# ZhongchuanSun/scikit-recommender

Measured on AMD Instinct MI355X. Metric: train interactions/sec + eval users/sec (HR@10/NDCG@10) at 1/2/4/8 MI355X, higher is better.
Workload: dtype f32; 1 GPU; BASELINE configs[1]: BPRMF d=64, synthetic 1000000-user/100000-item/50000000-interaction (MovieLens-shaped), exact-stream sampler + fused BPR step + dense Adam; eval = fused MFMA top-10; users=1000000, items=100000, train_interactions=48383462, batch_per_gpu=1024, global_batch=1024

## Files before the change

scikit-recommender_amd/csrc/bpr_fused.hip:

```cpp
#include "adam_math.h"

#include <cstdlib>

using namespace skr;

namespace {

constexpr int BPR_WAVES = 4;

constexpr int FUSED_SLOT_BITS = 20;
constexpr int FUSED_PRE = 7;

struct FusedRow {
    float p, m, v, g;
};

__device__ __forceinline__ void fused_advance(FusedRow& r, int prev1, int s_from, int s_to, const AdamBlockArgs& a, int ck) {
    if (prev1 > 0)
        adam_grad_run(r.p, r.g, r.m, r.v, a, prev1 - 1, s_to, ck);
    else
        adam_zero_run(r.p, r.m, r.v, a, s_from, s_to, ck);
}

struct FusedWork {
    float *wp, *wm, *wv, *g;
    int64_t cap;
};

__global__ __launch_bounds__(BPR_WAVES * 64) void bpr_fused_step_kernel(
    const float* __restrict__ P, const float* __restrict__ M, const float* __restrict__ V, int64_t n_par, FusedWork w,
    const int32_t* __restrict__ u_ids, const int32_t* __restrict__ i_ids, const int32_t* __restrict__ j_ids,
    const int32_t* __restrict__ meta, int n, int64_t ublk0, int64_t iblk0, int64_t bblk0, int s_now, AdamBlockArgs a,
    float reg, float* __restrict__ loss, int loss_slots, int dbg, const float* __restrict__ pre) {
    __shared__ float s_loss[BPR_WAVES], s_l2[BPR_WAVES];
    if (!(dbg & 16)) __builtin_amdgcn_s_setprio(3);
    const int lane = threadIdx.x & 63, wv = threadIdx.x >> 6;
    const AdamChainArgs ca = adam_chain_args(a);
    float acc_loss = 0.0f, acc_l2 = 0.0f;
    for (int b = blockIdx.x * BPR_WAVES + wv; b < n; b += gridDim.x * BPR_WAVES) {
        const int64_t u = u_ids[b], i = i_ids[b], j = j_ids[b];
        int32_t mt[5];
        int64_t blk[5] = {ublk0 + u, iblk0 + i, iblk0 + j, bblk0 + (i >> 6), bblk0 + (j >> 6)};
#pragma unroll
        for (int r = 0; r < 5; ++r) mt[r] = __builtin_amdgcn_readfirstlane(meta[static_cast<int64_t>(r) * n + b]);
        FusedRow row[5];
        int from[5];
#pragma unroll
        for (int r = 0; r < 5; ++r) {
            const int64_t slot = mt[r] & ((1 << FUSED_SLOT_BITS) - 1);
            int n0 = (mt[r] >> FUSED_SLOT_BITS) & 7;
            row[r] = FusedRow{1.0f, 0.0f, 0.0f, 0.0f};
            from[r] = (mt[r] >> 24) & 0x7f;
            if (n0 == FUSED_PRE) {
                const int64_t e = slot * 64 + lane;
                row[r].p = pre[e];
                row[r].m = pre[w.cap * 64 + e];
                row[r].v = pre[2 * w.cap * 64 + e];
                from[r] = s_now;
                mt[r] &= ~(7 << FUSED_SLOT_BITS);
                n0 = 0;
            } else if (((mt[r] >> 24) & 0x7f) == 0) {
                const int64_t e = blk[r] * 64 + lane;
                if (e < n_par) {
                    row[r].p = P[e];
                    row[r].m = M[e];
                    row[r].v = V[e];
                }
            } else {
                const int64_t e = ((n0 & 1) * w.cap + slot) * 64 + lane;
                row[r].p = w.wp[e];
                row[r].m = w.wm[e];
                row[r].v = w.wv[e];
                row[r].g = w.g[(((n0 + 2) % 3) * w.cap + slot) * 64 + lane];
            }
        }
        if (!(dbg & 1)) {
#pragma unroll
            for (int r = 0; r < 5; ++r) {
                const int prev1 = (mt[r] >> 24) & 0x7f;
                const AdamRowState o = chain_advance(row[r].p, row[r].g, row[r].m, row[r].v, prev1, from[r], s_now,
                                                     r < 3 ? FC_STEP_ROW : FC_STEP_BIAS, ca);
                row[r].p = o.p, row[r].m = o.m, row[r].v = o.v;
            }
        }
        if (!(dbg & 4)) {
#pragma unroll
            for (int r = 0; r < 5; ++r) {
                if ((mt[r] >> 23) & 1) {
                    const int64_t slot = mt[r] & ((1 << FUSED_SLOT_BITS) - 1);
                    const int n0 = (mt[r] >> FUSED_SLOT_BITS) & 7;
                    const int64_t e = (((n0 + 1) & 1) * w.cap + slot) * 64 + lane;
                    w.wp[e] = row[r].p;
                    w.wm[e] = row[r].m;
                    w.wv[e] = row[r].v;
                    w.g[(((n0 + 1) % 3) * w.cap + slot) * 64 + lane] = 0.0f;
                }
            }
        }
        const float pu = row[0].p, qi = row[1].p, qj = row[2].p;
        const float bi = __shfl(row[3].p, static_cast<int>(i & 63)), bj = __shfl(row[4].p, static_cast<int>(j & 63));
        const float xi = skr::wave_sum(pu * qi) + bi, xj = skr::wave_sum(pu * qj) + bj;
        const float x = xi - xj;
        const float z = expf(-fabsf(x));
        const float l = -(fminf(0.0f, x) - log1pf(z));
        const float sig_neg = (x >= 0.0f) ? z / (1.0f + z) : 1.0f / (1.0f + z);
        const float c = -sig_neg;
        float sq = skr::wave_sum(pu * pu + qi * qi + qj * qj);
        float* gcur[5];
#pragma unroll
        for (int r = 0; r < 5; ++r) {
            const int64_t slot = mt[r] & ((1 << FUSED_SLOT_BITS) - 1);
            const int n0 = (mt[r] >> FUSED_SLOT_BITS) & 7;
            gcur[r] = w.g + ((n0 % 3) * w.cap + slot) * 64;
        }
        if (!(dbg & 2)) {
            const float gu = c * (qi - qj) + reg * pu, gi = c * pu + reg * qi, gj = -c * pu + reg * qj;
            if (mt[0] < 0) gcur[0][lane] = gu; else atomicAdd(&gcur[0][lane], gu);
            if (mt[1] < 0) gcur[1][lane] = gi; else atomicAdd(&gcur[1][lane], gi);
            if (mt[2] < 0) gcur[2][lane] = gj; else atomicAdd(&gcur[2][lane], gj);
        }
        sq += bi * bi + bj * bj;
        if (lane == 0 && !(dbg & 2)) {
            atomicAdd(&gcur[3][i & 63], c + reg * bi);
            atomicAdd(&gcur[4][j & 63], -c + reg * bj);
        }
        acc_loss += l;
        acc_l2 += 0.5f * sq;
    }
    if (lane == 0) {
        s_loss[wv] = acc_loss;
        s_l2[wv] = acc_l2;
    }
    __syncthreads();
    if (threadIdx.x == 0 && !(dbg & 8)) {
        float x = 0.0f, y = 0.0f;
        for (int q = 0; q < BPR_WAVES; ++q) {
            x += s_loss[q];
            y += s_l2[q];
        }
        const int sl = 2 * (static_cast<int>(blockIdx.x) % loss_slots);
        atomicAdd(&loss[sl], x);
        atomicAdd(&loss[sl + 1], y);
    }
}

__global__ __launch_bounds__(256) void bpr_fused_pre_kernel(const float* __restrict__ P, const float* __restrict__ M,
                                                            const float* __restrict__ V, int64_t n_par, float* __restrict__ pre,
                                                            int64_t cap, const int32_t* __restrict__ slot_blk,
                                                            const int32_t* __restrict__ slot_fin, const int32_t* __restrict__ n_slots,
                                                            AdamBlockArgs a, const int32_t* __restrict__ tag_prev,
                                                            int32_t tag_prev_value) {
    const int lane = threadIdx.x & 63;
    const int64_t slot = blockIdx.x * 4 + (threadIdx.x >> 6);
    if (slot >= *n_slots) return;
    const int64_t blk = slot_blk[slot];
    const int first = (slot_fin[slot] >> 16) & 0xff;
    if (first == 0 || tag_prev[blk] == tag_prev_value) return;
    const int64_t e = blk * 64 + lane;
    FusedRow r{1.0f, 0.0f, 0.0f, 0.0f};
    if (e < n_par) { r.p = P[e]; r.m = M[e]; r.v = V[e]; }
    fused_advance(r, 0, 0, first, a, FC_PRE);
    const int64_t o = slot * 64 + lane;
    pre[o] = r.p;
    pre[cap * 64 + o] = r.m;
    pre[2 * cap * 64 + o] = r.v;
}

__global__ __launch_bounds__(256) void bpr_fused_end_kernel(float* __restrict__ P, float* __restrict__ M, float* __restrict__ V,
                                                            int64_t n_par, FusedWork w, const int32_t* __restrict__ slot_blk,
                                                            const int32_t* __restrict__ slot_fin,
                                                            const int32_t* __restrict__ n_slots, AdamBlockArgs a,
                                                            const int32_t* __restrict__ tag_next, int32_t tag_next_value, int which) {
    const int lane = threadIdx.x & 63;
    const int64_t slot0 = 2 * (static_cast<int64_t>(blockIdx.x) * 4 + __builtin_amdgcn_readfirstlane(threadIdx.x >> 6));
    const int64_t n = *n_slots;
    if (slot0 >= n) return;
    FusedRow r[2];
    int64_t e[2];
    int last[2];
    bool live[2];
#pragma unroll
    for (int h = 0; h < 2; ++h) {
        const int64_t slot = slot0 + h;
        live[h] = slot < n;
        e[h] = 0, last[h] = 0;
        r[h] = FusedRow{1.0f, 0.0f, 0.0f, 0.0f};
        if (!live[h]) continue;
        const int64_t blk = slot_blk[slot];
        if (which != 0 && ((tag_next[blk] == tag_next_value) != (which == 1))) {
            live[h] = false;
            continue;
        }
        const int fin = slot_fin[slot], nn = fin & 7;
        last[h] = (fin >> 8) & 0xff;
        e[h] = blk * 64 + lane;
        if (e[h] < n_par) {
            const int64_t o = ((nn & 1) * w.cap + slot) * 64 + lane;
            r[h].p = w.wp[o];
            r[h].m = w.wm[o];
            r[h].v = w.wv[o];
            r[h].g = w.g[(((nn + 2) % 3) * w.cap + slot) * 64 + lane];
        }
    }
    if (live[0] && live[1]) {
        bool ord[2];
#pragma unroll
        for (int h = 0; h < 2; ++h) {
            adam_moments(r[h].g, r[h].m, r[h].v, a);
            ord[h] = __builtin_amdgcn_ballot_w64(!lane_ordinary(r[h].m, r[h].v, a)) == 0;
        }
        if (ord[0] && ord[1]) {
            const int hi = last[0] > last[1] ? last[0] : last[1];
#pragma unroll
            for (int h = 0; h < 2; ++h) adam_grad_finish(r[h].p, r[h].m, r[h].v, a, last[h], hi + 1, FC_END, true);
            f32x2 p2{r[0].p, r[1].p}, m2{r[0].m, r[1].m}, v2{r[0].v, r[1].v};
            adam_pair_run(p2, m2, v2, a, hi + 1, a.k);
            r[0].p = p2.x, r[0].m = m2.x, r[0].v = v2.x;
            r[1].p = p2.y, r[1].m = m2.y, r[1].v = v2.y;
            if (a.stats && lane == 0) atomicAdd(&a.stats[FC_END_PAIRED], 2ull);
        } else {
#pragma unroll
            for (int h = 0; h < 2; ++h) adam_grad_finish(r[h].p, r[h].m, r[h].v, a, last[h], a.k, FC_END, ord[h]);
            if (a.stats && lane == 0) atomicAdd(&a.stats[FC_END_SINGLE], 2ull);
        }
    } else {
#pragma unroll
        for (int h = 0; h < 2; ++h) {
            if (!live[h]) continue;
            adam_grad_run(r[h].p, r[h].g, r[h].m, r[h].v, a, last[h], a.k, FC_END);
            if (a.stats && lane == 0) atomicAdd(&a.stats[FC_END_SINGLE], 1ull);
        }
    }
#pragma unroll
    for (int h = 0; h < 2; ++h) {
        if (!live[h]) continue;
        if (e[h] < n_par) {
            P[e[h]] = r[h].p;
            M[e[h]] = r[h].m;
            V[e[h]] = r[h].v;
        }
#pragma unroll
        for (int q = 0; q < 3; ++q) w.g[(q * w.cap + slot0 + h) * 64 + lane] = 0.0f;
    }
}

struct FusedPlanArgs {
    const int32_t *u, *i, *j;
    int k, b;
    int64_t ublk0, iblk0, bblk0;
    unsigned long long *named, *claimed, *shared;
    int32_t *slot_of, *meta, *slot_block, *slot_fin, *n_slots;
    const int32_t* tag_prev;
    int32_t tag_prev_value;
};

__device__ __forceinline__ void fused_plan_refs(const FusedPlanArgs& a, int64_t t, int64_t blk[5]) {
    const int64_t u = a.u[t], i = a.i[t], j = a.j[t];
    blk[0] = a.ublk0 + u;
    blk[1] = a.iblk0 + i;
    blk[2] = a.iblk0 + j;
    blk[3] = a.bblk0 + (i >> 6);
    blk[4] = a.bblk0 + (j >> 6);
}

template <int PASS>
__global__ __launch_bounds__(256) void fused_plan_kernel(FusedPlanArgs a) {
    const int64_t t = blockIdx.x * 256ll + threadIdx.x;
    if (PASS == 0 && t == 0) *a.n_slots = 0;
    if (t >= static_cast<int64_t>(a.k) * a.b) return;
    const int s = static_cast<int>(t / a.b);
    const int64_t col = t - static_cast<int64_t>(s) * a.b;
    int64_t blk[5];
    fused_plan_refs(a, t, blk);
    const unsigned long long bit = 1ull << s;
#pragma unroll
    for (int r = 0; r < 5; ++r) {
        const int64_t e = (static_cast<int64_t>(s) * 5 + r) * a.b + col;
        if (PASS == 0) {
            atomicOr(&a.named[blk[r]], bit);
            a.slot_block[e] = -1;
        } else if (PASS == 1) {
            const bool owner = (atomicOr(&a.claimed[blk[r]], bit) & bit) == 0;
            if (!owner) atomicOr(&a.shared[blk[r]], bit);
            a.meta[e] = owner ? (1 << 23) : 0;
            const unsigned long long mask = a.named[blk[r]];
            const bool draws = owner && (mask & (bit - 1)) == 0;
            const unsigned long long db = __ballot(draws);
            int base = 0;
            if (db) {
                const int leader = __ffsll(static_cast<long long>(db)) - 1;
                if (static_cast<int>(threadIdx.x & 63) == leader) base = atomicAdd(a.n_slots, __popcll(db));
                base = __shfl(base, leader);
            }
            if (draws) {
                const int slot = base + __popcll(db & ((1ull << (threadIdx.x & 63)) - 1ull));
                a.slot_of[blk[r]] = slot;
                a.slot_block[slot] = static_cast<int32_t>(blk[r]);
                a.slot_fin[slot] = (__popcll(mask) % 6) | ((63 - __clzll(static_cast<long long>(mask))) << 8) | (s << 16);
            }
        } else if (PASS == 2) {
            const unsigned long long below = a.named[blk[r]] & (bit - 1);
            const int n0 = __popcll(below), prev1 = below ? 64 - __clzll(static_cast<long long>(below)) : 0;
            const int sole = (a.shared[blk[r]] & bit) ? 0 : 1;
            const bool pre = a.tag_prev && below == 0 && s > 0 && a.tag_prev[blk[r]] != a.tag_prev_value;
            a.meta[e] = a.meta[e] | a.slot_of[blk[r]] | ((pre ? FUSED_PRE : n0 % 6) << FUSED_SLOT_BITS) | (prev1 << 24) |
                        static_cast<int32_t>(static_cast<uint32_t>(sole) << 31);
        } else {
            a.named[blk[r]] = 0;
            a.claimed[blk[r]] = 0;
            a.shared[blk[r]] = 0;
        }
    }
}

}

extern "C" {

static const AdamBlockArgs& fused_block_args(float lr, float beta1, float beta2, float eps, int64_t step_t0, int k) {
    struct Key {
        float lr, b1, b2, eps;
        int64_t t0;
        int k;
    };
    thread_local Key key{0, 0, 0, 0, -1, 0};
    thread_local AdamBlockArgs a{};
    if (key.lr != lr || key.b1 != beta1 || key.b2 != beta2 || key.eps != eps || key.t0 != step_t0 || key.k != k) {
        a = AdamBlockArgs{};
        adam_shared_fields(a, beta1, beta2, eps);
        a.k = k;
        adam_block_scalars(a, lr, beta1, beta2, step_t0, k, false);
        adam_block_thresholds(a, lr, beta1, beta2, eps, k);
        key = Key{lr, beta1, beta2, eps, step_t0, k};
    }
    a.stats = fused_stats_buffer();
    return a;
}

static FusedWork fused_work(float* d_work, int64_t cap) {
    const int64_t plane = cap * 64;
    return FusedWork{d_work, d_work + 2 * plane, d_work + 4 * plane, d_work + 6 * plane, cap};
}

int skr_bpr_fused_step(const float* d_p, const float* d_m, const float* d_v, int64_t n, float* d_work, int64_t cap,
                       const int32_t* d_u, const int32_t* d_i, const int32_t* d_j, const int32_t* d_meta, int n_batch,
                       int64_t user_block0, int64_t item_block0, int64_t bias_block0, float lr, float beta1, float beta2,
                       float eps, int64_t step_t0, int k, int s, float reg, float* d_loss64, void* stream) {
    return skr_bpr_fused_step2(d_p, d_m, d_v, n, d_work, cap, d_u, d_i, d_j, d_meta, n_batch, user_block0, item_block0, bias_block0, lr,
                               beta1, beta2, eps, step_t0, k, s, reg, d_loss64, nullptr, stream);
}

int skr_bpr_fused_step2(const float* d_p, const float* d_m, const float* d_v, int64_t n, float* d_work, int64_t cap,
                        const int32_t* d_u, const int32_t* d_i, const int32_t* d_j, const int32_t* d_meta, int n_batch,
                        int64_t user_block0, int64_t item_block0, int64_t bias_block0, float lr, float beta1, float beta2,
                        float eps, int64_t step_t0, int k, int s, float reg, float* d_loss64, const float* d_pre, void* stream) {
    SKR_REQUIRE(d_p && d_m && d_v && d_work && d_u && d_i && d_j && d_meta && d_loss64, "skr_bpr_fused_step: NULL argument");
    SKR_REQUIRE(n >= 0 && n_batch >= 0 && cap >= 1 && cap <= (1 << FUSED_SLOT_BITS), "skr_bpr_fused_step: need 1 <= cap <= 2^%d",
                FUSED_SLOT_BITS);
    SKR_REQUIRE(step_t0 >= 0 && k >= 1 && k <= AB_KMAX && s >= 0 && s < k, "skr_bpr_fused_step: need 0 <= s < k <= %d", AB_KMAX);
    SKR_REQUIRE(user_block0 >= 0 && item_block0 >= 0 && bias_block0 >= 0, "skr_bpr_fused_step: bad table offsets");
    if (n_batch == 0) return SKR_OK;
    const AdamBlockArgs& a = fused_block_args(lr, beta1, beta2, eps, step_t0, k);
    static const int dbg = [] { const char* e = getenv("SKR_FUSED_DBG"); return e ? atoi(e) : 0; }();
    int blocks = (n_batch + BPR_WAVES - 1) / BPR_WAVES;
    if (blocks > 256 * 16) blocks = 256 * 16;
    hipLaunchKernelGGL(bpr_fused_step_kernel, dim3(blocks), dim3(BPR_WAVES * 64), 0, skr::as_stream(stream), d_p, d_m, d_v, n,
                       fused_work(d_work, cap), d_u, d_i, d_j, d_meta, n_batch, user_block0, item_block0, bias_block0, s, a, reg,
                       d_loss64, SKR_LOSS_SLOTS, dbg, d_pre);
    SKR_LAUNCH_CHECK();
    return SKR_OK;
}

int skr_bpr_fused_plan(const int32_t* d_u, const int32_t* d_i, const int32_t* d_j, int n_batch, int k, int64_t user_block0,
                       int64_t item_block0, int64_t bias_block0, int64_t n_flat_blocks, void* d_scratch, int32_t* d_meta,
                       int32_t* d_slot_block, int32_t* d_slot_fin, int32_t* d_n_slots, void* stream) {
    return skr_bpr_fused_plan2(d_u, d_i, d_j, n_batch, k, user_block0, item_block0, bias_block0, n_flat_blocks, d_scratch, d_meta,
                               d_slot_block, d_slot_fin, d_n_slots, nullptr, 0, stream);
}

int skr_bpr_fused_plan2(const int32_t* d_u, const int32_t* d_i, const int32_t* d_j, int n_batch, int k, int64_t user_block0,
                        int64_t item_block0, int64_t bias_block0, int64_t n_flat_blocks, void* d_scratch, int32_t* d_meta,
                        int32_t* d_slot_block, int32_t* d_slot_fin, int32_t* d_n_slots, const int32_t* d_tag_prev,
                        int32_t tag_prev_value, void* stream) {
    SKR_REQUIRE(d_u && d_i && d_j && d_scratch && d_meta && d_slot_block && d_slot_fin && d_n_slots, "skr_bpr_fused_plan: NULL argument");
    SKR_REQUIRE(n_batch >= 1 && k >= 1 && k <= AB_KMAX && static_cast<int64_t>(k) * 5 * n_batch <= (1 << FUSED_SLOT_BITS),
                "skr_bpr_fused_plan: need 1 <= k <= %d and k * 5 * n_batch <= 2^%d", AB_KMAX, FUSED_SLOT_BITS);
    SKR_REQUIRE(user_block0 >= 0 && item_block0 >= 0 && bias_block0 >= 0 && n_flat_blocks >= 1 && n_flat_blocks < INT32_MAX,
                "skr_bpr_fused_plan: bad table offsets");
    SKR_REQUIRE((reinterpret_cast<uintptr_t>(d_scratch) & 7) == 0, "skr_bpr_fused_plan: scratch must be 8-byte aligned");
    FusedPlanArgs a;
    a.u = d_u, a.i = d_i, a.j = d_j;
    a.k = k, a.b = n_batch;
    a.ublk0 = user_block0, a.iblk0 = item_block0, a.bblk0 = bias_block0;
    a.named = static_cast<unsigned long long*>(d_scratch);
    a.claimed = a.named + n_flat_blocks;
    a.shared = a.claimed + n_flat_blocks;
    a.slot_of = reinterpret_cast<int32_t*>(a.shared + n_flat_blocks);
    a.meta = d_meta, a.slot_block = d_slot_block, a.slot_fin = d_slot_fin, a.n_slots = d_n_slots;
    a.tag_prev = d_tag_prev, a.tag_prev_value = tag_prev_value;
    const dim3 grid(static_cast<unsigned>((static_cast<int64_t>(k) * n_batch + 255) / 256)), wg(256);
    hipLaunchKernelGGL(fused_plan_kernel<0>, grid, wg, 0, skr::as_stream(stream), a);
    hipLaunchKernelGGL(fused_plan_kernel<1>, grid, wg, 0, skr::as_stream(stream), a);
    hipLaunchKernelGGL(fused_plan_kernel<2>, grid, wg, 0, skr::as_stream(stream), a);
    hipLaunchKernelGGL(fused_plan_kernel<3>, grid, wg, 0, skr::as_stream(stream), a);
    SKR_LAUNCH_CHECK();
    return SKR_OK;
}

int skr_bpr_fused_pre(const float* d_p, const float* d_m, const float* d_v, int64_t n, float* d_pre, int64_t cap,
                      const int32_t* d_slot_block, const int32_t* d_slot_fin, const int32_t* d_n_slots, float lr, float beta1,
                      float beta2, float eps, int64_t step_t0, int k, const int32_t* d_tag_prev, int32_t tag_prev_value,
                      void* stream) {
    SKR_REQUIRE(d_p && d_m && d_v && d_pre && d_slot_block && d_slot_fin && d_n_slots && d_tag_prev, "skr_bpr_fused_pre: NULL argument");
    SKR_REQUIRE(n >= 0 && cap >= 1 && cap <= (1 << FUSED_SLOT_BITS), "skr_bpr_fused_pre: need 1 <= cap <= 2^%d", FUSED_SLOT_BITS);
    SKR_REQUIRE(step_t0 >= 0 && k >= 1 && k <= AB_KMAX, "skr_bpr_fused_pre: need 1 <= k <= %d", AB_KMAX);
    AdamBlockArgs a{};
    adam_shared_fields(a, beta1, beta2, eps);
    a.k = k;
    adam_block_scalars(a, lr, beta1, beta2, step_t0, k, false);
    adam_block_thresholds(a, lr, beta1, beta2, eps, k);
    a.stats = fused_stats_buffer();
    hipLaunchKernelGGL(bpr_fused_pre_kernel, dim3(static_cast<unsigned>((cap + 3) / 4)), dim3(256), 0, skr::as_stream(stream), d_p, d_m,
                       d_v, n, d_pre, cap, d_slot_block, d_slot_fin, d_n_slots, a, d_tag_prev, tag_prev_value);
    SKR_LAUNCH_CHECK();
    return SKR_OK;
}

int skr_bpr_fused_end(float* d_p, float* d_m, float* d_v, int64_t n, float* d_work, int64_t cap, const int32_t* d_slot_block,
                      const int32_t* d_slot_fin, const int32_t* d_n_slots, float lr, float beta1, float beta2, float eps,
                      int64_t step_t0, int k, const int32_t* d_tag_next, int32_t tag_next_value, int which, void* stream) {
    SKR_REQUIRE(d_p && d_m && d_v && d_work && d_slot_block && d_slot_fin && d_n_slots, "skr_bpr_fused_end: NULL argument");
    SKR_REQUIRE(n >= 0 && cap >= 1 && cap <= (1 << FUSED_SLOT_BITS), "skr_bpr_fused_end: need 1 <= cap <= 2^%d", FUSED_SLOT_BITS);
    SKR_REQUIRE(step_t0 >= 0 && k >= 1 && k <= AB_KMAX, "skr_bpr_fused_end: need 1 <= k <= %d", AB_KMAX);
    SKR_REQUIRE(which >= 0 && which <= 2 && (which == 0 || d_tag_next), "skr_bpr_fused_end: which must be 0, or 1 / 2 with the next block's tags");
    const AdamBlockArgs& a = fused_block_args(lr, beta1, beta2, eps, step_t0, k);
    hipLaunchKernelGGL(bpr_fused_end_kernel, dim3(static_cast<unsigned>((cap + 7) / 8)), dim3(256), 0, skr::as_stream(stream), d_p,
                       d_m, d_v, n, fused_work(d_work, cap), d_slot_block, d_slot_fin, d_n_slots, a, d_tag_next, tag_next_value, which);
    SKR_LAUNCH_CHECK();
    return SKR_OK;
}

int skr_bpr_fused_block(float* d_p, float* d_m, float* d_v, int64_t n, float* d_work, int64_t cap, const int32_t* d_u,
                        const int32_t* d_i, const int32_t* d_j, const int32_t* d_meta, int n_batch, int64_t user_block0,
                        int64_t item_block0, int64_t bias_block0, float lr, float beta1, float beta2, float eps, int64_t step_t0,
                        int k, float reg, float* d_loss64, int64_t loss_stride_floats, const int32_t* d_slot_block,
                        const int32_t* d_slot_fin, const int32_t* d_n_slots, const int32_t* d_tag_next, int32_t tag_next_value,
                        void* stream) {
    return skr_bpr_fused_block2(d_p, d_m, d_v, n, d_work, cap, d_u, d_i, d_j, d_meta, n_batch, user_block0, item_block0, bias_block0, lr,
                                beta1, beta2, eps, step_t0, k, reg, d_loss64, loss_stride_floats, d_slot_block, d_slot_fin, d_n_slots,
                                d_tag_next, tag_next_value, nullptr, stream);
}

int skr_bpr_fused_block2(float* d_p, float* d_m, float* d_v, int64_t n, float* d_work, int64_t cap, const int32_t* d_u,
                         const int32_t* d_i, const int32_t* d_j, const int32_t* d_meta, int n_batch, int64_t user_block0,
                         int64_t item_block0, int64_t bias_block0, float lr, float beta1, float beta2, float eps, int64_t step_t0,
                         int k, float reg, float* d_loss64, int64_t loss_stride_floats, const int32_t* d_slot_block,
                         const int32_t* d_slot_fin, const int32_t* d_n_slots, const int32_t* d_tag_next, int32_t tag_next_value,
                         const float* d_pre, void* stream) {
    SKR_REQUIRE(k >= 1 && k <= AB_KMAX && n_batch >= 0 && loss_stride_floats >= 0, "skr_bpr_fused_block: bad shape");
    for (int s = 0; s < k; ++s) {
        const int64_t o = static_cast<int64_t>(s) * n_batch;
        const int rc = skr_bpr_fused_step2(d_p, d_m, d_v, n, d_work, cap, d_u + o, d_i + o, d_j + o, d_meta + 5 * o, n_batch, user_block0,
                                           item_block0, bias_block0, lr, beta1, beta2, eps, step_t0, k, s, reg,
                                           d_loss64 + s * loss_stride_floats, d_pre, stream);
        if (rc != SKR_OK) return rc;
    }
    return skr_bpr_fused_end(d_p, d_m, d_v, n, d_work, cap, d_slot_block, d_slot_fin, d_n_slots, lr, beta1, beta2, eps, step_t0, k,
                             d_tag_next, tag_next_value, d_tag_next ? 1 : 0, stream);
}

}
```

Before: 58.53 million train interactions/s.

## Compute per-row gather addresses lane-parallel and prefetch next sample's ids and metadata

```diff
diff --git a/scikit-recommender_amd/csrc/bpr_fused.hip b/scikit-recommender_amd/csrc/bpr_fused.hip
--- a/scikit-recommender_amd/csrc/bpr_fused.hip
+++ b/scikit-recommender_amd/csrc/bpr_fused.hip
@@ -21,6 +21,8 @@
     else
         adam_zero_run(r.p, r.m, r.v, a, s_from, s_to, ck);
 }
+
+typedef const float __attribute__((address_space(1)))* GlobalFloats;
 
 struct FusedWork {
     float *wp, *wm, *wv, *g;
@@ -33,53 +35,78 @@
     const int32_t* __restrict__ meta, int n, int64_t ublk0, int64_t iblk0, int64_t bblk0, int s_now, AdamBlockArgs a,
     float reg, float* __restrict__ loss, int loss_slots, int dbg, const float* __restrict__ pre) {
     __shared__ float s_loss[BPR_WAVES], s_l2[BPR_WAVES];
+    const int lane = threadIdx.x & 63, wv = threadIdx.x >> 6;
+    const int lr = lane < 16 ? lane >> 2 : 4, lq = lane & 3;
+    const int32_t* my_ids = lr == 0 ? u_ids : (lr & 1) ? i_ids : j_ids;
+    const int32_t* my_meta = meta + static_cast<int64_t>(lr) * n;
+    const int b0 = blockIdx.x * BPR_WAVES + wv, b_step = gridDim.x * BPR_WAVES;
+    int32_t next_id = my_ids[b0 < n ? b0 : n - 1], next_mt = my_meta[b0 < n ? b0 : n - 1];
+    const AdamChainArgs ca = adam_chain_args(a);
+    asm volatile("" ::"s"(P), "s"(M), "s"(V), "s"(n_par), "s"(w.wp), "s"(w.wm), "s"(w.wv), "s"(w.g), "s"(w.cap), "s"(pre), "s"(loss));
+    asm volatile("" ::"s"(ublk0), "s"(iblk0), "s"(bblk0), "s"(s_now), "s"(reg), "s"(loss_slots), "s"(dbg), "s"(ca.stats), "s"(ca.first_unit));
+    asm volatile("" ::"s"(ca.one_minus_b1), "s"(ca.b2), "s"(ca.one_minus_b2), "s"(ca.eps), "s"(ca.rest_eps), "s"(ca.rest_b2k), "s"(ca.fast_vlo),
+                 "s"(ca.fast_mlo), "s"(ca.fast_mhi));
     if (!(dbg & 16)) __builtin_amdgcn_s_setprio(3);
-    const int lane = threadIdx.x & 63, wv = threadIdx.x >> 6;
-    const AdamChainArgs ca = adam_chain_args(a);
     float acc_loss = 0.0f, acc_l2 = 0.0f;
-    for (int b = blockIdx.x * BPR_WAVES + wv; b < n; b += gridDim.x * BPR_WAVES) {
-        const int64_t u = u_ids[b], i = i_ids[b], j = j_ids[b];
+    for (int b = b0; b < n; b += b_step) {
+        const int32_t my_id = next_id;
+        int32_t my_mt = next_mt;
+        int my_lim, my_from;
+        uint64_t my_addr;
+        {
+            const int64_t blk = lr == 0 ? ublk0 + my_id : lr < 3 ? iblk0 + my_id : bblk0 + (my_id >> 6);
+            const int64_t slot = my_mt & ((1 << FUSED_SLOT_BITS) - 1);
+            const int n0 = (my_mt >> FUSED_SLOT_BITS) & 7, prev1 = (my_mt >> 24) & 0x7f;
+            const bool is_pre = n0 == FUSED_PRE, is_dense = !is_pre && prev1 == 0;
+            const int64_t tail = n_par - 1 - blk * 64;
+            const bool in_dense = is_dense && tail >= 0;
+            my_lim = is_dense && tail < 63 ? (tail < 0 ? -1 : static_cast<int>(tail)) : 63;
+            my_from = is_pre ? s_now : prev1;
+            if (is_pre) my_mt &= ~(7 << FUSED_SLOT_BITS);
+            const uint64_t b_dense = reinterpret_cast<uint64_t>(lq == 0 ? P : lq == 1 ? M : V);
+            const uint64_t b_work = reinterpret_cast<uint64_t>(lq == 0 ? w.wp : lq == 1 ? w.wm : lq == 2 ? w.wv : w.g);
+            const uint64_t b_pre = reinterpret_cast<uint64_t>(pre) + static_cast<uint64_t>(lq * w.cap) * 256;
+            const int64_t e_work = lq == 3 ? ((n0 + 2) % 3) * w.cap + slot : (n0 & 1) * w.cap + slot;
+            my_addr = lq == 3 ? b_work + e_work * 256 : is_pre ? b_pre + slot * 256 : in_dense ? b_dense + blk * 256 : b_work + e_work * 256;
+        }
+        const int64_t i = __builtin_amdgcn_readlane(my_id, 4), j = __builtin_amdgcn_readlane(my_id, 8);
         int32_t mt[5];
-        int64_t blk[5] = {ublk0 + u, iblk0 + i, iblk0 + j, bblk0 + (i >> 6), bblk0 + (j >> 6)};
-#pragma unroll
-        for (int r = 0; r < 5; ++r) mt[r] = __builtin_amdgcn_readfirstlane(meta[static_cast<int64_t>(r) * n + b]);
         FusedRow row[5];
         int from[5];
+        int lim[5];
 #pragma unroll
         for (int r = 0; r < 5; ++r) {
-            const int64_t slot = mt[r] & ((1 << FUSED_SLOT_BITS) - 1);
-            int n0 = (mt[r] >> FUSED_SLOT_BITS) & 7;
-            row[r] = FusedRow{1.0f, 0.0f, 0.0f, 0.0f};
-            from[r] = (mt[r] >> 24) & 0x7f;
-            if (n0 == FUSED_PRE) {
-                const int64_t e = slot * 64 + lane;
-                row[r].p = pre[e];
-                row[r].m = pre[w.cap * 64 + e];
-                row[r].v = pre[2 * w.cap * 64 + e];
-                from[r] = s_now;
-                mt[r] &= ~(7 << FUSED_SLOT_BITS);
-                n0 = 0;
-            } else if (((mt[r] >> 24) & 0x7f) == 0) {
-                const int64_t e = blk[r] * 64 + lane;
-                if (e < n_par) {
-                    row[r].p = P[e];
-                    row[r].m = M[e];
-                    row[r].v = V[e];
-                }
-            } else {
-                const int64_t e = ((n0 & 1) * w.cap + slot) * 64 + lane;
-                row[r].p = w.wp[e];
-                row[r].m = w.wm[e];
-                row[r].v = w.wv[e];
-                row[r].g = w.g[(((n0 + 2) % 3) * w.cap + slot) * 64 + lane];
-            }
-        }
-        if (!(dbg & 1)) {
-#pragma unroll
-            for (int r = 0; r < 5; ++r) {
+            mt[r] = __builtin_amdgcn_readlane(my_mt, 4 * r);
+            from[r] = __builtin_amdgcn_readlane(my_from, 4 * r);
+            lim[r] = __builtin_amdgcn_readlane(my_lim, 4 * r);
+            const uint32_t lo = lane < lim[r] ? lane : (lim[r] < 0 ? 0 : lim[r]);
+            GlobalFloats src[4];
+#pragma unroll
+            for (int q = 0; q < 4; ++q)
+                src[q] = reinterpret_cast<GlobalFloats>(
+                    static_cast<uint64_t>(static_cast<uint32_t>(__builtin_amdgcn_readlane(static_cast<int>(my_addr), 4 * r + q))) |
+                    static_cast<uint64_t>(static_cast<uint32_t>(__builtin_amdgcn_readlane(static_cast<int>(my_addr >> 32), 4 * r + q))) << 32);
+            row[r].p = src[0][lo];
+            row[r].m = src[1][lo];
+            row[r].v = src[2][lo];
+            row[r].g = __hip_atomic_load(src[3] + lane, __ATOMIC_RELAXED, __HIP_MEMORY_SCOPE_WAVEFRONT);
+        }
+        next_id = my_ids[b + b_step < n ? b + b_step : n - 1], next_mt = my_meta[b + b_step < n ? b + b_step : n - 1];
+        AdamChainArgs cb = ca;
+        asm volatile("" : "+v"(cb.t_bc2));
+        const float rb = __builtin_amdgcn_rcpf(cb.t_bc2);
+        cb.t_rbc2 = __builtin_fmaf(__builtin_fmaf(-cb.t_bc2, rb, 1.0f), rb, rb);
+#pragma unroll
+        for (int r = 0; r < 5; ++r) {
+            const bool past = lane > lim[r];
+            row[r].p = past ? 1.0f : row[r].p;
+            row[r].m = past ? 0.0f : row[r].m;
+            row[r].v = past ? 0.0f : row[r].v;
+            row[r].g = ((mt[r] >> 24) & 0x7f) != 0 ? row[r].g : 0.0f;
+            if (!(dbg & 1)) {
                 const int prev1 = (mt[r] >> 24) & 0x7f;
                 const AdamRowState o = chain_advance(row[r].p, row[r].g, row[r].m, row[r].v, prev1, from[r], s_now,
-                                                     r < 3 ? FC_STEP_ROW : FC_STEP_BIAS, ca);
+                                                     r < 3 ? FC_STEP_ROW : FC_STEP_BIAS, cb);
                 row[r].p = o.p, row[r].m = o.m, row[r].v = o.v;
             }
         }
```

Result: faster. 60.91 million train interactions/s (median of 6 runs) (+4.1%).
